# lmb-freiburg/demon

Hardware: NVIDIA H100
Metric: image_pairs_per_sec_256x192 (higher is better)
Workload: dtype tf32x3

## Files before the change

### demon_b200/csrc/conv_tc_halo.cu

```cuda
#include <cuda.h>

#include <algorithm>
#include <cstring>
#include <memory>
#include <mutex>
#include <vector>

#include "conv_tc.cuh"
#include "conv_tc_ptx.cuh"
#include "wgmma_tf32.cuh"

namespace demon {

namespace {

constexpr int kRing = 4;
constexpr int kThreads = 384;
constexpr int kConsumerWarps = 8;
constexpr int kMaxAStages = 4;
constexpr int kTileH = 16, kTileW = 8;
constexpr int kMaxPlanes = 4;
constexpr int kPlanSms = 132;
constexpr int kSmemBudget = 224 * 1024;
constexpr int kMaxDynSmem = 226 * 1024;
// ... 30 lines not shown
  int w_resident;
  int cls_bytes;
  int n_tile, nsplit;
  int mode;
  const unsigned char* w;
  float* out;
  int out_pitch, Ho, Wo, Hfull, Wfull, osy, osx, Cout;
  int cls_ooy[4], cls_oox[4];
  const float* bias;
  int leaky;
  int* err;
  long long* timing;
};

struct HaloMaps {
  CUtensorMap m[kMaxPlanes];
};

__device__ __forceinline__ void wait_t(uint32_t bar, uint32_t parity, int* err, long long& acc) {
  if (mbar_try(bar, parity)) return;
  const long long t0 = clock64();
  for (;;) {
    if (mbar_try(bar, parity)) break;
    if (clock64() - t0 > kTimeoutCycles || *reinterpret_cast<volatile int*>(err) != 0) {
      atomicExch(err, 1);
      break;
    }
  }
  acc += clock64() - t0;
}

__device__ __forceinline__ int fast_div(int x, int d, uint32_t mul) { return mul ? (int)__umulhi((uint32_t)x, mul) : x; }

template <bool PER_TAP>
__device__ __forceinline__ void halo_decode_tile(const HaloParams& p, int tile, int& nt, int& n, int& y0, int& x0) {
  int m = fast_div(tile, p.n_tiles, p.mul_n_tiles);
  nt = tile - m * p.n_tiles;
  const int m1 = fast_div(m, p.tiles_x, p.mul_tiles_x);
  const int xb = m - m1 * p.tiles_x;
  n = fast_div(m1, p.tiles_y, p.mul_tiles_y);
  const int yb = m1 - n * p.tiles_y;
  if (PER_TAP) { n *= p.tb; y0 = yb * p.th; x0 = xb * p.tw; }
  else { y0 = yb * kTileH; x0 = xb * kTileW; }
}

template <int N, int MODE>
__device__ __forceinline__ void issue_block(float* acc, const uint32_t* hi, const uint32_t* lo, uint32_t wb) {
  const uint64_t w_hi = wgmma_desc_sw128(wb);
  const uint64_t w_lo = wgmma_desc_sw128(wb + N * 128u);
#pragma unroll
  for (int j = 0; j < 4; ++j) {
    if (MODE == 2) {
      Wgmma<N>::mma(acc, hi[4 * j], hi[4 * j + 1], hi[4 * j + 2], hi[4 * j + 3], w_lo + (uint64_t)(2 * j));
      Wgmma<N>::mma(acc, lo[4 * j], lo[4 * j + 1], lo[4 * j + 2], lo[4 * j + 3], w_hi + (uint64_t)(2 * j));
    }
    Wgmma<N>::mma(acc, hi[4 * j], hi[4 * j + 1], hi[4 * j + 2], hi[4 * j + 3], w_hi + (uint64_t)(2 * j));
  }
}

template <bool PER_TAP, bool CIN8, int MODE, int N, int NCLS>
__global__ void __launch_bounds__(kThreads, 1) conv_tc_halo_kernel(const __grid_constant__ HaloMaps maps, const HaloParams p) {
  extern __shared__ __align__(1024) unsigned char smem_raw[];
  unsigned char* smem = reinterpret_cast<unsigned char*>((reinterpret_cast<uintptr_t>(smem_raw) + 1023) & ~(uintptr_t)1023);
  __shared__ __align__(8) uint64_t bars[2 * kMaxAStages + 2 * kRing + 1];

  const int warp = threadIdx.x >> 5;
  const int lane = threadIdx.x & 31;
  const uint32_t afull0 = smem_u32(&bars[0]), aempty0 = smem_u32(&bars[kMaxAStages]);
  const uint32_t wfull0 = smem_u32(&bars[2 * kMaxAStages]), wempty0 = smem_u32(&bars[2 * kMaxAStages + kRing]);
  const uint32_t wres_bar = smem_u32(&bars[2 * kMaxAStages + 2 * kRing]);
  const int a_stage_bytes = p.a_region_bytes;
  unsigned char* w_ring = smem + (size_t)p.sa * a_stage_bytes;

  if (warp == 0 && lane == 0) {
    for (int i = 0; i < p.nplanes; ++i) asm volatile("prefetch.tensormap [%0];" ::"l"(&maps.m[i]) : "memory");
    for (int s = 0; s < kMaxAStages; ++s) {
      mbar_init(afull0 + 8 * s, 1);
      mbar_init(aempty0 + 8 * s, kConsumerWarps);
    }
    for (int s = 0; s < kRing; ++s) {
      mbar_init(wfull0 + 8 * s, 1);
      mbar_init(wempty0 + 8 * s, kConsumerWarps);
    }
    mbar_init(wres_bar, 1);
    fence_barrier_init();
  }
  __syncthreads();
  const bool timed = p.timing != nullptr;
  pdl_launch_dependents();

  if (warp < 4) {
    asm volatile("setmaxnreg.dec.sync.aligned.u32 40;");
    if (warp != 0 || !elect_one_sync()) return;
    long long w_aempty = 0, w_wempty = 0;
    const long long t_begin = clock64();
    if (p.w_resident) {
      const uint32_t total = (uint32_t)(p.k_chunks * p.w_chunk_bytes);
      mbar_expect_tx(wres_bar, total);
      for (int kc = 0; kc < p.k_chunks; ++kc)
        bulk_load(smem_u32(w_ring + (size_t)kc * p.w_chunk_bytes), p.w + (size_t)kc * p.w_chunk_bytes, (uint32_t)p.w_chunk_bytes, wres_bar);
    }
    uint32_t a_bytes = 0;
    for (int i = 0; i < p.nplanes; ++i) a_bytes += (uint32_t)p.planes[i].bytes;
    int sa = 0, slot = 0;
    uint32_t pa = 0, use = 0;
    pdl_wait();
    for (int item = blockIdx.x; item < p.total_items; item += gridDim.x) {
      const int tile = fast_div(item, p.ksplit, p.mul_ksplit);
      const int kc0 = (item - tile * p.ksplit) * p.kc_split;
      int nt, n, y0, x0;
      halo_decode_tile<PER_TAP>(p, tile, nt, n, y0, x0);
      const unsigned char* wsrc = p.w + ((size_t)nt * p.k_chunks + kc0) * p.w_chunk_bytes;
      for (int kc = kc0; kc < kc0 + p.kc_split; ++kc, wsrc += p.w_chunk_bytes) {
        if (!PER_TAP) {
          wait_t(aempty0 + 8 * sa, pa ^ 1, p.err, w_aempty);
          const uint32_t abase = smem_u32(smem + (size_t)sa * a_stage_bytes);
          mbar_expect_tx(afull0 + 8 * sa, a_bytes);
          for (int i = 0; i < p.nplanes; ++i) {
            const HaloPlane& pl = p.planes[i];
            tma_load_5d(abase + pl.smem_off, &maps.m[i], afull0 + 8 * sa, pl.c_off + kc * 32, x0 + pl.qx_min, pl.ry, y0 + pl.qy_min, n);
          }
          if (++sa == p.sa) { sa = 0; pa ^= 1; }
        }
        for (int t = 0; t < p.nsteps; ++t) {
          if (PER_TAP) {
            wait_t(aempty0 + 8 * sa, pa ^ 1, p.err, w_aempty);
            mbar_expect_tx(afull0 + 8 * sa, 128u * 128u);
            tma_load_5d(smem_u32(smem + (size_t)sa * a_stage_bytes), &maps.m[0], afull0 + 8 * sa, p.tap_c[t] + kc * 32, x0 + p.tap_qx[t],
                        p.tap_ry[t], y0 + p.tap_qy[t], n);
            if (++sa == p.sa) { sa = 0; pa ^= 1; }
          }
          if (!p.w_resident) {
            wait_t(wempty0 + 8 * slot, use ^ 1, p.err, w_wempty);
            const uint32_t bytes = (uint32_t)p.st_wbytes[t];
            mbar_expect_tx(wfull0 + 8 * slot, bytes);
            bulk_load(smem_u32(w_ring + (size_t)slot * p.w_stage_bytes), wsrc + p.st_woff[t], bytes, wfull0 + 8 * slot);
            if (++slot == kRing) { slot = 0; use ^= 1; }
          }
        }
      }
    }
    if (timed) { p.timing[blockIdx.x * 16 + 0] = w_aempty; p.timing[blockIdx.x * 16 + 1] = w_wempty; p.timing[blockIdx.x * 16 + 8] = clock64() - t_begin; }
    return;
  }

  asm volatile("setmaxnreg.inc.sync.aligned.u32 232;");
  const int wg = (warp >> 2) - 1;
  const int wq = warp & 3;
  const int g = lane >> 2, tq = lane & 3;
  const int m0 = 64 * wg + 16 * wq + g;
  int pos_y[2], pos_x[2], pos_n[2];
#pragma unroll
  for (int h = 0; h < 2; ++h) {
    const int m = m0 + 8 * h;
    pos_x[h] = PER_TAP ? (m % p.tw) : (m & 7);
    pos_y[h] = PER_TAP ? ((m / p.tw) % p.th) : (m >> 3);
    pos_n[h] = PER_TAP ? (m / (p.tw * p.th)) : 0;
  }
  const float slope = p.leaky ? 0.1f : 1.0f;
  const uint32_t w_ring_u = smem_u32(w_ring);
  long long w_afull = 0, w_wfull = 0;
  const long long t_begin = clock64();
  int sa = 0, slot = 0, l_res = 0;
  uint32_t pa = 0, use = 0;
  if (p.w_resident) wait_t(wres_bar, 0u, p.err, w_wfull);
  pdl_wait();
  float acc[NCLS][N / 2];
  for (int item = blockIdx.x; item < p.total_items; item += gridDim.x) {
    const int tile = fast_div(item, p.ksplit, p.mul_ksplit);
    const int z = item - tile * p.ksplit;
    int nt, n, y0, x0;
    halo_decode_tile<PER_TAP>(p, tile, nt, n, y0, x0);
#pragma unroll
    for (int k = 0; k < NCLS; ++k)
#pragma unroll
      for (int i = 0; i < N / 2; ++i) acc[k][i] = 0.f;
    l_res = 0;
    for (int kc = 0; kc < p.kc_split; ++kc) {
      uint32_t abase = 0;
      if (!PER_TAP) {
        wait_t(afull0 + 8 * sa, pa, p.err, w_afull);
        abase = smem_u32(smem + (size_t)sa * a_stage_bytes);
      }
      for (int t = 0; t < p.nsteps; ++t) {
        if (PER_TAP) {
          wait_t(afull0 + 8 * sa, pa, p.err, w_afull);
          abase = smem_u32(smem + (size_t)sa * a_stage_bytes);
        }
        float v[2][8];
#pragma unroll
        for (int h = 0; h < 2; ++h) {
          if (CIN8) {
            const int rt = 4 * t + tq;
            const int pi = (rt < p.ntaps_real) ? p.g_plane[rt] : -1;
            float4 a = make_float4(0.f, 0.f, 0.f, 0.f), b = a;
            if (pi >= 0) {
              const HaloPlane& pl = p.planes[pi];
              const uint32_t px = abase + (uint32_t)(pl.smem_off + p.g_aoff[rt] + (pos_y[h] * pl.cols + pos_x[h]) * 32);
              a = lds128(px); b = lds128(px + 16);
            }
            v[h][0] = a.x; v[h][1] = a.y; v[h][2] = a.z; v[h][3] = a.w; v[h][4] = b.x; v[h][5] = b.y; v[h][6] = b.z; v[h][7] = b.w;
          } else {
            uint32_t row;
            if (PER_TAP) {
              row = abase + (uint32_t)((m0 + 8 * h) * 128);
            } else {
              const HaloPlane& pl = p.planes[p.st_plane[t]];
              row = abase + (uint32_t)(pl.smem_off + p.st_aoff[t] + (pos_y[h] * pl.cols + pos_x[h]) * 128);
            }
            const uint32_t phase = (row >> 7) & 7u;
            const float4 a = lds128(row + (((uint32_t)(2 * tq) ^ phase) << 4));
            const float4 b = lds128(row + (((uint32_t)(2 * tq + 1) ^ phase) << 4));
            v[h][0] = a.x; v[h][1] = a.y; v[h][2] = a.z; v[h][3] = a.w; v[h][4] = b.x; v[h][5] = b.y; v[h][6] = b.z; v[h][7] = b.w;
          }
        }
        uint32_t hi[16], lo[16];
#pragma unroll
        for (int j = 0; j < 4; ++j) {
          const float f[4] = {v[0][2 * j], v[1][2 * j], v[0][2 * j + 1], v[1][2 * j + 1]};
#pragma unroll
          for (int e = 0; e < 4; ++e) {
            const uint32_t u = __float_as_uint(f[e]);
            hi[4 * j + e] = (MODE == 2) ? (u & 0xFFFFE000u) : u;
            lo[4 * j + e] = __float_as_uint(f[e] - __uint_as_float(u & 0xFFFFE000u));
          }
        }
        uint32_t wb;
        if (p.w_resident) {
          wb = w_ring_u + (uint32_t)(l_res++) * (uint32_t)p.w_stage_bytes;
        } else {
          wait_t(wfull0 + 8 * slot, use, p.err, w_wfull);
          wb = w_ring_u + (uint32_t)slot * (uint32_t)p.w_stage_bytes;
        }
#pragma unroll
        for (int k = 0; k < NCLS; ++k)
#pragma unroll
          for (int i = 0; i < N / 2; ++i) reg_fence(acc[k][i]);
        wgmma_fence();
        if (NCLS == 1) {
          issue_block<N, MODE>(acc[0], hi, lo, wb);
        } else {
          const uint32_t cm = (uint32_t)p.st_cmask[t];
#pragma unroll
          for (int k = 0; k < NCLS; ++k)
            if (cm & (1u << k)) {
              issue_block<N, MODE>(acc[k], hi, lo, wb);
              wb += (uint32_t)p.cls_bytes;
            }
        }
        wgmma_commit();
        wgmma_wait0();
#pragma unroll
        for (int k = 0; k < NCLS; ++k)
#pragma unroll
          for (int i = 0; i < N / 2; ++i) reg_fence(acc[k][i]);
        __syncwarp();
        if (lane == 0) {
          if (!p.w_resident) mbar_arrive(wempty0 + 8 * slot);
          if (PER_TAP) mbar_arrive(aempty0 + 8 * sa);
        }
        if (!p.w_resident && ++slot == kRing) { slot = 0; use ^= 1; }
        if (PER_TAP && ++sa == p.sa) { sa = 0; pa ^= 1; }
      }
      if (!PER_TAP) {
        __syncwarp();
        if (lane == 0) mbar_arrive(aempty0 + 8 * sa);
        if (++sa == p.sa) { sa = 0; pa ^= 1; }
      }
    }
    float* tile_out = p.out + (size_t)z * p.part_stride + ((size_t)(n * p.Hfull + y0 * p.osy) * p.Wfull + x0 * p.osx) * p.out_pitch;
    const int cbase = nt * N;
#pragma unroll
    for (int k = 0; k < NCLS; ++k) {
      if (k >= p.nclass) break;
      float* cls_out = tile_out + (size_t)(p.cls_ooy[k] * p.Wfull + p.cls_oox[k]) * p.out_pitch;
#pragma unroll
      for (int h = 0; h < 2; ++h) {
        if (y0 + pos_y[h] >= p.Ho || x0 + pos_x[h] >= p.Wo || n + pos_n[h] >= p.B) continue;
        float* orow = cls_out + ((size_t)(pos_n[h] * p.Hfull + pos_y[h] * p.osy) * p.Wfull + pos_x[h] * p.osx) * p.out_pitch;
#pragma unroll
        for (int i = 0; i < N / 8; ++i) {
          const int col = cbase + 8 * i + 2 * tq;
          if (col >= p.Cout) continue;
          const float2 b = p.bias ? __ldg(reinterpret_cast<const float2*>(p.bias + col)) : make_float2(0.f, 0.f);
          float2 o;
          o.x = acc[k][4 * i + 2 * h] + b.x;
          o.y = acc[k][4 * i + 2 * h + 1] + b.y;
          o.x = fmaxf(slope * o.x, o.x); o.y = fmaxf(slope * o.y, o.y);
          *reinterpret_cast<float2*>(orow + col) = o;
        }
      }
    }
  }
  if (timed && threadIdx.x == 128) { p.timing[blockIdx.x * 16 + 6] = w_afull; p.timing[blockIdx.x * 16 + 3] = w_wfull; p.timing[blockIdx.x * 16 + 9] = clock64() - t_begin; }
}

__global__ void __launch_bounds__(256) halo_splitk_reduce_kernel(const float* __restrict__ part, long long part_stride, int ksplit,
                                                                 float* __restrict__ out, int out_pitch, int cpitch, int Cout, long long npix,
                                                                 const float* __restrict__ bias, int leaky) {
  pdl_launch_dependents();
  pdl_wait();
  const int c4n = cpitch >> 2;
  const long long total = npix * c4n;
  const float slope = leaky ? 0.1f : 1.0f;
  for (long long i = (long long)blockIdx.x * 256 + threadIdx.x; i < total; i += (long long)gridDim.x * 256) {
    const long long pix = i / c4n;
    const int c = (int)(i - pix * c4n) * 4;
    if (c >= Cout) continue;
    float4 acc = __ldg(reinterpret_cast<const float4*>(bias + c));
    for (int z = 0; z < ksplit; ++z) {
      const float4 v = *reinterpret_cast<const float4*>(part + (size_t)z * part_stride + (size_t)pix * cpitch + c);
      acc.x += v.x; acc.y += v.y; acc.z += v.z; acc.w += v.w;
    }
    acc.x = fmaxf(slope * acc.x, acc.x); acc.y = fmaxf(slope * acc.y, acc.y);
    acc.z = fmaxf(slope * acc.z, acc.z); acc.w = fmaxf(slope * acc.w, acc.w);
    *reinterpret_cast<float4*>(out + (size_t)pix * out_pitch + c) = acc;
  }
}

int floor_div_h(int a, int b) { return (a >= 0) ? a / b : -((-a + b - 1) / b); }

}

struct HaloPlan {
  HaloParams prm;
  HaloMaps maps;
  int smem_bytes;
  int st_tap[kMaxTaps][4];
};

static int pow2_ceil_h(int v) { int r = 1; while (r < v) r <<= 1; return r; }
static int popcount4(int m) { return (m & 1) + ((m >> 1) & 1) + ((m >> 2) & 1) + ((m >> 3) & 1); }

struct ShiftStep { int ry, rx, qy, qx, cmask, tap[4]; };

static bool halo_build(const ConvProblem* probs, int nclass, int nsplit, HaloPlan& plan, bool force_per_tap) {
  const ConvProblem& p = probs[0];
  HaloParams& prm = plan.prm;
  const int budget = kSmemBudget;
  struct Cand { int max_cls, n_cap; };
  std::vector<Cand> cands;
  for (int mc = nclass; mc >= 1; mc = (mc > 2 ? 2 : mc - 1)) cands.push_back({mc, 256});
  cands.push_back({1, 64});
  cands.push_back({1, 32});
  bool found = false;
  for (const Cand& cand : cands) {
    const int max_cls = cand.max_cls;
    memset(&prm, 0, sizeof(prm));
    memset(plan.st_tap, -1, sizeof(plan.st_tap));
    prm.nclass = nclass;
    prm.nsplit = nsplit;
    prm.cin8 = (p.Cin == 8) ? 1 : 0;
    const int px_bytes = prm.cin8 ? 32 : 128;
    prm.per_tap = (force_per_tap || (p.Ho % kTileH) != 0 || (p.Wo % kTileW) != 0) ? 1 : 0;
    if (prm.cin8 && (prm.per_tap || nclass != 1)) return false;
    std::vector<ShiftStep> steps;
    for (int c = 0; c < nclass; ++c)
      for (int i = 0; i < probs[c].ntaps; ++i) {
        const int qy = floor_div_h(probs[c].dy[i], p.sy), ry = probs[c].dy[i] - qy * p.sy;
        const int qx = floor_div_h(probs[c].dx[i], p.sx), rx = probs[c].dx[i] - qx * p.sx;
        int si = -1;
        for (size_t k = 0; k < steps.size(); ++k)
          if (steps[k].ry == ry && steps[k].rx == rx && steps[k].qy == qy && steps[k].qx == qx && !((steps[k].cmask >> c) & 1) &&
              popcount4(steps[k].cmask) < max_cls) { si = (int)k; break; }
        if (si < 0) { steps.push_back({ry, rx, qy, qx, 0, {-1, -1, -1, -1}}); si = (int)steps.size() - 1; }
        steps[si].cmask |= 1 << c;
        steps[si].tap[c] = i;
      }
    const int nreal = (int)steps.size();
    if (nreal > kMaxTaps) return false;
    int m_tiles = 0;
    if (prm.per_tap) {
      for (int t = 0; t < nreal; ++t) {
        prm.tap_qy[t] = steps[t].qy; prm.tap_ry[t] = steps[t].ry;
        prm.tap_qx[t] = steps[t].qx; prm.tap_c[t] = steps[t].rx * p.in_pitch;
      }
      prm.nplanes = 1;
      long best_tiles = -1;
      const int tw = std::min(128, pow2_ceil_h(p.Wo));
      for (int th = 1; th * tw <= 128; th <<= 1) {
        const int tb = 128 / (tw * th);
        const long tiles = (long)ceil_div(p.Wo, tw) * ceil_div(p.Ho, th) * ceil_div(p.B, tb);
        if (best_tiles < 0 || tiles <= best_tiles) {
          best_tiles = tiles;
          prm.tw = tw; prm.th = th; prm.tb = tb;
          prm.tiles_x = ceil_div(p.Wo, tw); prm.tiles_y = ceil_div(p.Ho, th); prm.tiles_b = ceil_div(p.B, tb);
        }
      }
      prm.planes[0].cols = prm.tw; prm.planes[0].rows = prm.th; prm.planes[0].bytes = 128 * 128;
      prm.a_region_bytes = 128 * 128;
      m_tiles = prm.tiles_x * prm.tiles_y * prm.tiles_b;
    } else {
      struct PInfo { int ry, rx, qy_min, qy_max, qx_min, qx_max; };
      std::vector<PInfo> pinfo;
      std::vector<int> step_plane(nreal);
      for (int t = 0; t < nreal; ++t) {
        int pi = -1;
        for (size_t k = 0; k < pinfo.size(); ++k)
          if (pinfo[k].ry == steps[t].ry && pinfo[k].rx == steps[t].rx) pi = (int)k;
        if (pi < 0) { pinfo.push_back({steps[t].ry, steps[t].rx, steps[t].qy, steps[t].qy, steps[t].qx, steps[t].qx}); pi = (int)pinfo.size() - 1; }
        PInfo& pl = pinfo[pi];
        pl.qy_min = std::min(pl.qy_min, steps[t].qy); pl.qy_max = std::max(pl.qy_max, steps[t].qy);
        pl.qx_min = std::min(pl.qx_min, steps[t].qx); pl.qx_max = std::max(pl.qx_max, steps[t].qx);
        step_plane[t] = pi;
      }
      if ((int)pinfo.size() > kMaxPlanes) return false;
      prm.nplanes = (int)pinfo.size();
      int off = 0;
      for (int i = 0; i < prm.nplanes; ++i) {
        HaloPlane& pl = prm.planes[i];
        pl.c_off = pinfo[i].rx * p.in_pitch; pl.ry = pinfo[i].ry;
        pl.qx_min = pinfo[i].qx_min; pl.qy_min = pinfo[i].qy_min;
        pl.cols = kTileW + pinfo[i].qx_max - pinfo[i].qx_min;
        pl.rows = kTileH + pinfo[i].qy_max - pinfo[i].qy_min;
        if (pl.cols > 256 || pl.rows > 256) return false;
        pl.bytes = pl.rows * pl.cols * px_bytes;
        pl.smem_off = off;
        off += (pl.bytes + 1023) / 1024 * 1024;
      }
      prm.a_region_bytes = off;
      for (int t = 0; t < nreal; ++t) {
        const HaloPlane& pl = prm.planes[step_plane[t]];
        prm.st_plane[t] = step_plane[t];
        prm.st_aoff[t] = ((steps[t].qy - pl.qy_min) * pl.cols + (steps[t].qx - pl.qx_min)) * px_bytes;
      }
      prm.tiles_x = ceil_div(p.Wo, kTileW); prm.tiles_y = ceil_div(p.Ho, kTileH); prm.tiles_b = p.B;
      m_tiles = prm.tiles_x * prm.tiles_y * p.B;
    }
    for (int t = 0; t < nreal; ++t) {
      prm.st_cmask[t] = steps[t].cmask;
      for (int c = 0; c < 4; ++c) plan.st_tap[t][c] = steps[t].tap[c];
    }
    prm.nsteps = nreal;
    if (prm.cin8) {
      prm.ntaps_real = nreal;
      for (int t = 0; t < nreal; ++t) { prm.g_plane[t] = prm.st_plane[t]; prm.g_aoff[t] = prm.st_aoff[t]; }
      prm.nsteps = (nreal + 3) / 4;
      for (int t = 0; t < prm.nsteps; ++t) { prm.st_plane[t] = 0; prm.st_aoff[t] = 0; prm.st_cmask[t] = 1; }
    }
    const int cout16 = (p.Cout + 15) / 16 * 16;
    int n_tile = std::min(pow2_ceil_h(std::max(cout16, 16)), std::min(nclass > 1 ? 64 : 128, cand.n_cap));
    while (n_tile >= 128 && (long)m_tiles * ceil_div(p.Cout, n_tile) < kPlanSms) n_tile /= 2;
    prm.mode = (nsplit == 1) ? 0 : 2;
    prm.n_tile = n_tile;
    prm.n_tiles = ceil_div(p.Cout, n_tile);
    prm.k_chunks = prm.cin8 ? 1 : p.Cin / 32;
    prm.cls_bytes = (nsplit == 3) ? n_tile * 256 : (n_tile * 128 + 1023) / 1024 * 1024;
    int woff = 0, wmax = 0;
    for (int t = 0; t < prm.nsteps; ++t) {
      prm.st_woff[t] = woff;
      prm.st_wbytes[t] = popcount4(prm.st_cmask[t]) * prm.cls_bytes;
      woff += prm.st_wbytes[t];
      wmax = std::max(wmax, prm.st_wbytes[t]);
    }
    prm.w_chunk_bytes = woff;
    prm.w_stage_bytes = wmax;
    const int w_total = prm.k_chunks * prm.w_chunk_bytes;
    prm.w_resident = 0;
    prm.w_region_bytes = kRing * wmax;
// ... 24 lines not shown
    for (int ks = 2; ks <= 8; ++ks) {
      if (prm.k_chunks % ks != 0 || prm.k_chunks / ks < 2) continue;
      const long c = cost(ks);
      if (c * 10 < best * 9 && c < cost(prm.ksplit)) prm.ksplit = ks;
    }
  }
  prm.kc_split = prm.k_chunks / prm.ksplit;
  prm.total_items = prm.total_tiles * prm.ksplit;
  prm.part_stride = 0;
  auto fd = [](int d) { return d <= 1 ? 0u : (uint32_t)((1ull << 32) / (uint64_t)d + 1ull); };
  prm.mul_n_tiles = fd(prm.n_tiles); prm.mul_tiles_x = fd(prm.tiles_x); prm.mul_tiles_y = fd(prm.tiles_y);
  prm.mul_ksplit = fd(prm.ksplit);
  if ((uint64_t)prm.total_items * (uint64_t)prm.ksplit >= (1ull << 32)) return false;
  if ((uint64_t)prm.total_tiles * (uint64_t)std::max(prm.n_tiles, std::max(prm.tiles_x, prm.tiles_y)) >= (1ull << 32)) return false;
  prm.out = p.out; prm.out_pitch = p.out_pitch; prm.Ho = p.Ho; prm.Wo = p.Wo; prm.Hfull = p.Hfull; prm.Wfull = p.Wfull;
  prm.osy = p.osy; prm.osx = p.osx; prm.Cout = p.Cout; prm.bias = p.bias; prm.leaky = p.leaky;
  for (int c = 0; c < nclass; ++c) { prm.cls_ooy[c] = probs[c].ooy; prm.cls_oox[c] = probs[c].oox; }
  return true;
}

static bool tc_shape_supported(const ConvProblem& p) {
  const bool cin8 = p.Cin == 8 && p.in_pitch == 8;
  if (!cin8 && (p.Cin < 32 || (p.Cin % 32) != 0)) return false;
  if (p.Cout < 16 || (p.Cout % 4) != 0) return false;
  if ((p.in_pitch % 4) != 0 || (p.out_pitch % 4) != 0) return false;
  if ((reinterpret_cast<uintptr_t>(p.in) & 15) != 0 || (reinterpret_cast<uintptr_t>(p.out) & 15) != 0) return false;
  if (p.sy < 1 || p.sx < 1 || (p.Hi % p.sy) != 0 || (p.Wi % p.sx) != 0) return false;
  if (p.ntaps < 1 || p.ntaps > kMaxTaps) return false;
  if (p.scale != nullptr) return false;
  if (p.Ho != p.Hi / p.sy || p.Wo != p.Wi / p.sx) return false;
  return true;
}

static bool tc_plan(const ConvProblem* probs, int nclass, int nsplit, HaloPlan& plan) {
  if (nclass < 1 || nclass > 4) return false;
  for (int c = 0; c < nclass; ++c) {
    if (!tc_shape_supported(probs[c])) return false;
    if (probs[c].in != probs[0].in || probs[c].Cout != probs[0].Cout || probs[c].sy != probs[0].sy || probs[c].sx != probs[0].sx) return false;
  }
  return halo_build(probs, nclass, nsplit, plan, false) || halo_build(probs, nclass, nsplit, plan, true);
}

static int nsplit_of(int precision) { return (precision == DEMON_PREC_TF32) ? 1 : 3; }

static bool encode_maps(const ConvProblem& p, HaloPlan& plan) {
  const HaloParams& prm = plan.prm;
  typedef CUresult (*EncodeTiledFn)(CUtensorMap*, CUtensorMapDataType, cuuint32_t, void*, const cuuint64_t*, const cuuint64_t*,
                                    const cuuint32_t*, const cuuint32_t*, CUtensorMapInterleave, CUtensorMapSwizzle,
                                    CUtensorMapL2promotion, CUtensorMapFloatOOBfill);
  void* fp = nullptr;
  cudaDriverEntryPointQueryResult qres;
  if (cudaGetDriverEntryPoint("cuTensorMapEncodeTiled", &fp, cudaEnableDefault, &qres) != cudaSuccess || qres != cudaDriverEntryPointSuccess)
    return false;
  EncodeTiledFn enc = reinterpret_cast<EncodeTiledFn>(fp);
  const cuuint64_t cp = (cuuint64_t)p.in_pitch;
  cuuint64_t gdim[5] = {(cuuint64_t)(p.sx - 1) * cp + (cuuint64_t)p.Cin, (cuuint64_t)(p.Wi / p.sx), (cuuint64_t)p.sy,
                        (cuuint64_t)(p.Hi / p.sy), (cuuint64_t)p.B};
  cuuint64_t gstr[4] = {(cuuint64_t)p.sx * cp * 4, (cuuint64_t)p.Wi * cp * 4, (cuuint64_t)p.sy * p.Wi * cp * 4,
                        (cuuint64_t)p.Hi * p.Wi * cp * 4};
  cuuint32_t estr[5] = {1, 1, 1, 1, 1};
  for (int i = 0; i < prm.nplanes; ++i) {
    cuuint32_t box[5] = {(cuuint32_t)(prm.cin8 ? 8 : 32), (cuuint32_t)prm.planes[i].cols, 1, (cuuint32_t)prm.planes[i].rows,
                         (cuuint32_t)(prm.per_tap ? prm.tb : 1)};
    CUresult r = enc(&plan.maps.m[i], CU_TENSOR_MAP_DATA_TYPE_FLOAT32, 5, const_cast<float*>(p.in), gdim, gstr, box, estr,
                     CU_TENSOR_MAP_INTERLEAVE_NONE, prm.cin8 ? CU_TENSOR_MAP_SWIZZLE_NONE : CU_TENSOR_MAP_SWIZZLE_128B,
                     CU_TENSOR_MAP_L2_PROMOTION_L2_256B, CU_TENSOR_MAP_FLOAT_OOB_FILL_NONE);
    if (r != CUDA_SUCCESS) return false;
  }
  for (int i = prm.nplanes; i < kMaxPlanes; ++i) plan.maps.m[i] = plan.maps.m[0];
  return true;
}

int tc_describe(const ConvProblem* probs, int nclass, int precision, char* buf, int buflen) {
  HaloPlan plan;
  if (!tc_plan(probs, nclass, nsplit_of(precision), plan)) return 0;
  const HaloParams& q = plan.prm;
  int n = snprintf(buf, buflen, "halo %s mode %d n_tile %d x%d steps %d x %d chunks sa %d a_stage %d w_slot %d smem %d tiles %d ksplit %d wres %d |",
                   q.per_tap ? "per-tap" : (q.cin8 ? "cin8" : "halo"), q.mode, q.n_tile, q.n_tiles, q.nsteps, q.k_chunks, q.sa,
                   q.a_region_bytes, q.w_stage_bytes, plan.smem_bytes, q.total_tiles, q.ksplit, q.w_resident);
  for (int t = 0; t < q.nsteps && n < buflen - 32; ++t)
    n += snprintf(buf + n, buflen - n, " [c%x w%d+%d]", q.st_cmask[t], q.st_woff[t], q.st_wbytes[t]);
  return n;
}

static float tf32_round_h(float x) {
  uint32_t u;
  memcpy(&u, &x, 4);
  if ((u & 0x7F800000u) == 0x7F800000u) return x;
  u += 0x00000FFFu + ((u >> 13) & 1u);
  u &= 0xFFFFE000u;
  float r;
  memcpy(&r, &u, 4);
  return r;
}

int tc_prepare(TcLayer& t, const ConvProblem* probs, const float* const* w_hosts, int nclass, int precision) {
  const ConvProblem& p = probs[0];
  const int nsplit = nsplit_of(precision);
  std::unique_ptr<HaloPlan> plan(new HaloPlan());
  if (!tc_plan(probs, nclass, nsplit, *plan)) return kTcNoPlan;
  if (!encode_maps(p, *plan)) return fail(DEMON_E_CUDA, "tc_prepare: tensor map encode failed");
  const HaloParams& prm = plan->prm;
  const size_t total = (size_t)prm.n_tiles * prm.k_chunks * prm.w_chunk_bytes;
  std::vector<unsigned char> packed(total, 0);
  for (int nt = 0; nt < prm.n_tiles; ++nt)
    for (int kc = 0; kc < prm.k_chunks; ++kc)
      for (int tt = 0; tt < prm.nsteps; ++tt) {
        int idx = 0;
        for (int cls = 0; cls < 4; ++cls) {
          if (!((prm.st_cmask[tt] >> cls) & 1)) continue;
          unsigned char* blk = packed.data() + ((size_t)nt * prm.k_chunks + kc) * prm.w_chunk_bytes + prm.st_woff[tt] + (size_t)idx * prm.cls_bytes;
          ++idx;
// ... 58 lines not shown
  if (s.device != dev) {
    s = TcDeviceState();
    s.device = dev;
    int sms = 0;
    cudaDeviceGetAttribute(&sms, cudaDevAttrMultiProcessorCount, dev);
    s.sms = sms > 0 ? sms : 132;
    if (cudaMalloc(&s.err_dev, sizeof(int)) == cudaSuccess) cudaMemset(s.err_dev, 0, sizeof(int));
    else s.err_dev = nullptr;
  }
  return s;
}

int tc_read_error_flag(bool clear) {
  TcDeviceState& ds = tc_device_state();
  if (!ds.err_dev) return 0;
  int v = 0;
  cudaMemcpy(&v, ds.err_dev, sizeof(int), cudaMemcpyDeviceToHost);
  if (v && clear) cudaMemset(ds.err_dev, 0, sizeof(int));
  return v;
}

static long long* g_timing_dev = nullptr;
void tc_halo_enable_timing(bool on) {
  if (on && !g_timing_dev) { cudaMalloc(&g_timing_dev, 256 * 16 * sizeof(long long)); }
  if (g_timing_dev) cudaMemset(g_timing_dev, 0, 256 * 16 * sizeof(long long));
  if (!on && g_timing_dev) { cudaFree(g_timing_dev); g_timing_dev = nullptr; }
}
int tc_halo_read_timing(long long* host, int nblocks) {
  if (!g_timing_dev) return -1;
  cudaMemcpy(host, g_timing_dev, (size_t)nblocks * 16 * sizeof(long long), cudaMemcpyDeviceToHost);
  return 0;
}

template <bool PER_TAP, bool CIN8, int MODE, int N, int NCLS>
static int launch_variant(const HaloPlan* plan, const HaloParams& prm, int grid, cudaStream_t stream) {
  TcDeviceState& ds = tc_device_state();
  static int attr_device = -1;
  if (attr_device != ds.device) {
    DEMON_CHECK_CUDA(cudaFuncSetAttribute(conv_tc_halo_kernel<PER_TAP, CIN8, MODE, N, NCLS>, cudaFuncAttributeMaxDynamicSharedMemorySize, kMaxDynSmem));
    attr_device = ds.device;
  }
  cudaError_t le = launch_pdl(conv_tc_halo_kernel<PER_TAP, CIN8, MODE, N, NCLS>, dim3(grid), dim3(kThreads), (size_t)plan->smem_bytes, stream, plan->maps, prm);
  if (le != cudaSuccess) return fail(DEMON_E_CUDA, "conv_tc_halo launch: %s", cudaGetErrorString(le));
  DEMON_LAUNCH_CHECK();
  return DEMON_OK;
}

template <bool PER_TAP, bool CIN8, int MODE, int NCLS>
static int launch_n(const HaloPlan* plan, const HaloParams& prm, int grid, cudaStream_t stream) {
  switch (prm.n_tile) {
    case 16: return launch_variant<PER_TAP, CIN8, MODE, 16, NCLS>(plan, prm, grid, stream);
    case 32: return launch_variant<PER_TAP, CIN8, MODE, 32, NCLS>(plan, prm, grid, stream);
    case 64: return launch_variant<PER_TAP, CIN8, MODE, 64, NCLS>(plan, prm, grid, stream);
    default: break;
  }
  if (NCLS == 1 && prm.n_tile == 128) return launch_variant<PER_TAP, CIN8, MODE, (NCLS == 1 ? 128 : 64), NCLS>(plan, prm, grid, stream);
  return fail(DEMON_E_STATE, "conv_tc_halo: no kernel for N tile %d with %d classes", prm.n_tile, prm.nclass);
}

template <bool PER_TAP, bool CIN8, int NCLS>
static int launch_mode(const HaloPlan* plan, const HaloParams& prm, int grid, cudaStream_t stream) {
  return prm.mode == 0 ? launch_n<PER_TAP, CIN8, 0, NCLS>(plan, prm, grid, stream) : launch_n<PER_TAP, CIN8, 2, NCLS>(plan, prm, grid, stream);
}

int conv_tc_launch(const TcLayer& t, const ConvProblem* probs, cudaStream_t stream) {
  const HaloPlan* plan = t.plan;
  HaloParams prm = plan->prm;
  prm.out = probs[0].out;
  prm.out_pitch = probs[0].out_pitch;
  TcDeviceState& ds = tc_device_state();
  if (!ds.err_dev) return fail(DEMON_E_CUDA, "tensor-core path: no error flag on device %d", ds.device);
  prm.err = ds.err_dev;
  prm.timing = g_timing_dev;
  const int cpitch = (prm.Cout + 3) / 4 * 4;
  const long long npix = (long long)prm.B * prm.Hfull * prm.Wfull;
  float* const final_out = prm.out;
  const int final_pitch = prm.out_pitch;
  if (prm.ksplit > 1) {
    if (!probs[0].partial) return fail(DEMON_E_STATE, "conv_tc_halo: split-K layer launched without a scratch buffer");
    prm.out = probs[0].partial;
    prm.out_pitch = cpitch;
    prm.part_stride = npix * cpitch;
    prm.bias = nullptr;
    prm.leaky = 0;
  }
  const int grid = std::min(prm.total_items, ds.sms);
  int rc;
  if (prm.cin8) rc = launch_mode<false, true, 1>(plan, prm, grid, stream);
  else if (prm.per_tap) rc = prm.nclass == 1 ? launch_mode<true, false, 1>(plan, prm, grid, stream) : launch_mode<true, false, 4>(plan, prm, grid, stream);
  else rc = prm.nclass == 1 ? launch_mode<false, false, 1>(plan, prm, grid, stream) : launch_mode<false, false, 4>(plan, prm, grid, stream);
  if (rc != DEMON_OK || prm.ksplit == 1) return rc;
  const long long total = npix * (cpitch / 4);
  const int blocks = (int)std::min<long long>((total + 255) / 256, (long long)ds.sms * 8);
  cudaError_t le = launch_pdl(halo_splitk_reduce_kernel, dim3(blocks), dim3(256), 0, stream, (const float*)probs[0].partial, prm.part_stride,
                              prm.ksplit, final_out, final_pitch, cpitch, prm.Cout, npix, plan->prm.bias, plan->prm.leaky);
  if (le != cudaSuccess) return fail(DEMON_E_CUDA, "halo_splitk_reduce launch: %s", cudaGetErrorString(le));
  DEMON_LAUNCH_CHECK();
  return DEMON_OK;
}

}
```

### demon_b200/csrc/conv_tc_ptx.cuh

```cuda
#pragma once
#include <cuda.h>
#include <cstdint>

namespace demon {
namespace {

constexpr long long kTimeoutCycles = 4000000000ll;

__device__ __forceinline__ uint32_t smem_u32(const void* p) { return (uint32_t)__cvta_generic_to_shared(p); }

__device__ __forceinline__ void mbar_init(uint32_t bar, uint32_t count) {
  asm volatile("mbarrier.init.shared::cta.b64 [%0], %1;" ::"r"(bar), "r"(count));
}
__device__ __forceinline__ void mbar_arrive(uint32_t bar) {
  asm volatile("{\n.reg .b64 st;\nmbarrier.arrive.shared::cta.b64 st, [%0];\n}" ::"r"(bar) : "memory");
}
__device__ __forceinline__ void mbar_expect_tx(uint32_t bar, uint32_t bytes) {
  asm volatile("{\n.reg .b64 st;\nmbarrier.arrive.expect_tx.shared::cta.b64 st, [%0], %1;\n}" ::"r"(bar), "r"(bytes) : "memory");
}
__device__ __forceinline__ bool mbar_try(uint32_t bar, uint32_t parity) {
  uint32_t done;
  asm volatile(
      "{\n.reg .pred p;\n"
      "mbarrier.try_wait.parity.shared::cta.b64 p, [%1], %2;\n"
      "selp.u32 %0, 1, 0, p;\n}"
      : "=r"(done)
      : "r"(bar), "r"(parity)
      : "memory");
  return done != 0;
}
__device__ __forceinline__ void fence_barrier_init() { asm volatile("fence.mbarrier_init.release.cluster;" ::: "memory"); }
__device__ __forceinline__ void tma_load_5d(uint32_t dst, const CUtensorMap* map, uint32_t bar, int c0, int c1, int c2, int c3, int c4) {
  asm volatile(
      "cp.async.bulk.tensor.5d.shared::cluster.global.mbarrier::complete_tx::bytes [%0], [%1, {%3, %4, %5, %6, %7}], [%2];"
      ::"r"(dst), "l"(map), "r"(bar), "r"(c0), "r"(c1), "r"(c2), "r"(c3), "r"(c4)
      : "memory");
}
__device__ __forceinline__ void bulk_load(uint32_t dst, const void* src, uint32_t bytes, uint32_t bar) {
  asm volatile("cp.async.bulk.shared::cluster.global.mbarrier::complete_tx::bytes [%0], [%1], %2, [%3];" ::"r"(dst), "l"(src),
               "r"(bytes), "r"(bar)
               : "memory");
}
__device__ __forceinline__ void wgmma_fence() { asm volatile("wgmma.fence.sync.aligned;" ::: "memory"); }
__device__ __forceinline__ void wgmma_commit() { asm volatile("wgmma.commit_group.sync.aligned;" ::: "memory"); }
__device__ __forceinline__ void wgmma_wait0() { asm volatile("wgmma.wait_group.sync.aligned 0;" ::: "memory"); }
__device__ __forceinline__ void reg_fence(float& x) { asm volatile("" : "+f"(x)::"memory"); }

__device__ __forceinline__ uint64_t wgmma_desc_sw128(uint32_t smem_addr) {
  uint64_t d = 0;
  d |= (uint64_t)((smem_addr & 0x3FFFF) >> 4);
  d |= (uint64_t)1 << 16;
  d |= (uint64_t)(1024 >> 4) << 32;
  d |= (uint64_t)1 << 62;
  return d;
}

__device__ __forceinline__ bool elect_one_sync() {
  uint32_t pred;
  asm volatile("{\n.reg .b32 rx;\n.reg .pred px;\nelect.sync rx|px, 0xffffffff;\nselp.b32 %0, 1, 0, px;\n}" : "=r"(pred));
  return pred != 0;
}

__device__ __forceinline__ float4 lds128(uint32_t addr) {
  float4 v;
  asm volatile("ld.shared.v4.f32 {%0, %1, %2, %3}, [%4];" : "=f"(v.x), "=f"(v.y), "=f"(v.z), "=f"(v.w) : "r"(addr));
  return v;
}
}
}
```

Before: 2050.

## Add two-block-wide halo tiles so each consumer reuses weights across two M blocks

Adds an MB=2 variant of the halo conv kernel in which each tile is twice as wide (16 columns). Each consumer warpgroup then keeps two 64-row accumulator sets and issues wgmma for both against the same weight descriptor, so every staged weight slice is reused across twice as many pixels. The planner picks this variant only for single-class, non-per-tap layers with N≤64 and enough tiles and pipeline stages. The cost is doubled accumulator and fragment registers, larger A stages that may reduce the stage count, and fewer tiles for load balancing.

New measurement: 2106, median of 6. 2.8% higher.

```diff
diff --git a/demon_b200/csrc/conv_tc_halo.cu b/demon_b200/csrc/conv_tc_halo.cu
--- a/demon_b200/csrc/conv_tc_halo.cu
+++ b/demon_b200/csrc/conv_tc_halo.cu
@@ -86,7 +86,7 @@
 
 __device__ __forceinline__ int fast_div(int x, int d, uint32_t mul) { return mul ? (int)__umulhi((uint32_t)x, mul) : x; }
 
-template <bool PER_TAP>
+template <bool PER_TAP, int TW>
 __device__ __forceinline__ void halo_decode_tile(const HaloParams& p, int tile, int& nt, int& n, int& y0, int& x0) {
   int m = fast_div(tile, p.n_tiles, p.mul_n_tiles);
   nt = tile - m * p.n_tiles;
@@ -95,7 +95,16 @@
   n = fast_div(m1, p.tiles_y, p.mul_tiles_y);
   const int yb = m1 - n * p.tiles_y;
   if (PER_TAP) { n *= p.tb; y0 = yb * p.th; x0 = xb * p.tw; }
-  else { y0 = yb * kTileH; x0 = xb * kTileW; }
+  else { y0 = yb * kTileH; x0 = xb * TW; }
+}
+
+template <int N, int MODE>
+__device__ __forceinline__ void issue_slice(float* acc, const uint32_t* hi, const uint32_t* lo, uint64_t w_hi, uint64_t w_lo, int j) {
+  if (MODE == 2) {
+    Wgmma<N>::mma(acc, hi[4 * j], hi[4 * j + 1], hi[4 * j + 2], hi[4 * j + 3], w_lo + (uint64_t)(2 * j));
+    Wgmma<N>::mma(acc, lo[4 * j], lo[4 * j + 1], lo[4 * j + 2], lo[4 * j + 3], w_hi + (uint64_t)(2 * j));
+  }
+  Wgmma<N>::mma(acc, hi[4 * j], hi[4 * j + 1], hi[4 * j + 2], hi[4 * j + 3], w_hi + (uint64_t)(2 * j));
 }
 
 template <int N, int MODE>
@@ -103,17 +112,13 @@
   const uint64_t w_hi = wgmma_desc_sw128(wb);
   const uint64_t w_lo = wgmma_desc_sw128(wb + N * 128u);
 #pragma unroll
-  for (int j = 0; j < 4; ++j) {
-    if (MODE == 2) {
-      Wgmma<N>::mma(acc, hi[4 * j], hi[4 * j + 1], hi[4 * j + 2], hi[4 * j + 3], w_lo + (uint64_t)(2 * j));
-      Wgmma<N>::mma(acc, lo[4 * j], lo[4 * j + 1], lo[4 * j + 2], lo[4 * j + 3], w_hi + (uint64_t)(2 * j));
-    }
-    Wgmma<N>::mma(acc, hi[4 * j], hi[4 * j + 1], hi[4 * j + 2], hi[4 * j + 3], w_hi + (uint64_t)(2 * j));
-  }
-}
-
-template <bool PER_TAP, bool CIN8, int MODE, int N, int NCLS>
+  for (int j = 0; j < 4; ++j) issue_slice<N, MODE>(acc, hi, lo, w_hi, w_lo, j);
+}
+
+template <bool PER_TAP, bool CIN8, int MODE, int N, int NCLS, int MB>
 __global__ void __launch_bounds__(kThreads, 1) conv_tc_halo_kernel(const __grid_constant__ HaloMaps maps, const HaloParams p) {
+  static_assert(MB == 1 || (MB == 2 && !PER_TAP && !CIN8 && NCLS == 1 && N <= 64), "MB = 2: one-class halo mode, N <= 64");
+  constexpr int TW = kTileW * MB;
   extern __shared__ __align__(1024) unsigned char smem_raw[];
   unsigned char* smem = reinterpret_cast<unsigned char*>((reinterpret_cast<uintptr_t>(smem_raw) + 1023) & ~(uintptr_t)1023);
   __shared__ __align__(8) uint64_t bars[2 * kMaxAStages + 2 * kRing + 1];
@@ -163,7 +168,7 @@
       const int tile = fast_div(item, p.ksplit, p.mul_ksplit);
       const int kc0 = (item - tile * p.ksplit) * p.kc_split;
       int nt, n, y0, x0;
-      halo_decode_tile<PER_TAP>(p, tile, nt, n, y0, x0);
+      halo_decode_tile<PER_TAP, TW>(p, tile, nt, n, y0, x0);
       const unsigned char* wsrc = p.w + ((size_t)nt * p.k_chunks + kc0) * p.w_chunk_bytes;
       for (int kc = kc0; kc < kc0 + p.kc_split; ++kc, wsrc += p.w_chunk_bytes) {
         if (!PER_TAP) {
@@ -203,14 +208,22 @@
   const int wq = warp & 3;
   const int g = lane >> 2, tq = lane & 3;
   const int m0 = 64 * wg + 16 * wq + g;
-  int pos_y[2], pos_x[2], pos_n[2];
-#pragma unroll
-  for (int h = 0; h < 2; ++h) {
-    const int m = m0 + 8 * h;
-    pos_x[h] = PER_TAP ? (m % p.tw) : (m & 7);
-    pos_y[h] = PER_TAP ? ((m / p.tw) % p.th) : (m >> 3);
-    pos_n[h] = PER_TAP ? (m / (p.tw * p.th)) : 0;
-  }
+  int pos_y[MB][2], pos_x[MB][2], pos_n[MB][2];
+#pragma unroll
+  for (int bk = 0; bk < MB; ++bk)
+#pragma unroll
+    for (int h = 0; h < 2; ++h) {
+      if (MB == 1) {
+        const int m = m0 + 8 * h;
+        pos_x[bk][h] = PER_TAP ? (m % p.tw) : (m & 7);
+        pos_y[bk][h] = PER_TAP ? ((m / p.tw) % p.th) : (m >> 3);
+        pos_n[bk][h] = PER_TAP ? (m / (p.tw * p.th)) : 0;
+      } else {
+        pos_x[bk][h] = g + 8 * h;
+        pos_y[bk][h] = 8 * wg + 4 * bk + wq;
+        pos_n[bk][h] = 0;
+      }
+    }
   const float slope = p.leaky ? 0.1f : 1.0f;
   const uint32_t w_ring_u = smem_u32(w_ring);
   long long w_afull = 0, w_wfull = 0;
@@ -219,14 +232,14 @@
   uint32_t pa = 0, use = 0;
   if (p.w_resident) wait_t(wres_bar, 0u, p.err, w_wfull);
   pdl_wait();
-  float acc[NCLS][N / 2];
+  float acc[NCLS * MB][N / 2];
   for (int item = blockIdx.x; item < p.total_items; item += gridDim.x) {
     const int tile = fast_div(item, p.ksplit, p.mul_ksplit);
     const int z = item - tile * p.ksplit;
     int nt, n, y0, x0;
-    halo_decode_tile<PER_TAP>(p, tile, nt, n, y0, x0);
-#pragma unroll
-    for (int k = 0; k < NCLS; ++k)
+    halo_decode_tile<PER_TAP, TW>(p, tile, nt, n, y0, x0);
+#pragma unroll
+    for (int k = 0; k < NCLS * MB; ++k)
 #pragma unroll
       for (int i = 0; i < N / 2; ++i) acc[k][i] = 0.f;
     l_res = 0;
@@ -241,44 +254,50 @@
           wait_t(afull0 + 8 * sa, pa, p.err, w_afull);
           abase = smem_u32(smem + (size_t)sa * a_stage_bytes);
         }
-        float v[2][8];
-#pragma unroll
-        for (int h = 0; h < 2; ++h) {
-          if (CIN8) {
-            const int rt = 4 * t + tq;
-            const int pi = (rt < p.ntaps_real) ? p.g_plane[rt] : -1;
-            float4 a = make_float4(0.f, 0.f, 0.f, 0.f), b = a;
-            if (pi >= 0) {
-              const HaloPlane& pl = p.planes[pi];
-              const uint32_t px = abase + (uint32_t)(pl.smem_off + p.g_aoff[rt] + (pos_y[h] * pl.cols + pos_x[h]) * 32);
-              a = lds128(px); b = lds128(px + 16);
+        float v[MB][2][8];
+#pragma unroll
+        for (int bk = 0; bk < MB; ++bk)
+#pragma unroll
+          for (int h = 0; h < 2; ++h) {
+            if (CIN8) {
+              const int rt = 4 * t + tq;
+              const int pi = (rt < p.ntaps_real) ? p.g_plane[rt] : -1;
+              float4 a = make_float4(0.f, 0.f, 0.f, 0.f), b = a;
+              if (pi >= 0) {
+                const HaloPlane& pl = p.planes[pi];
+                const uint32_t px = abase + (uint32_t)(pl.smem_off + p.g_aoff[rt] + (pos_y[bk][h] * pl.cols + pos_x[bk][h]) * 32);
+                a = lds128(px); b = lds128(px + 16);
+              }
+              v[bk][h][0] = a.x; v[bk][h][1] = a.y; v[bk][h][2] = a.z; v[bk][h][3] = a.w;
+              v[bk][h][4] = b.x; v[bk][h][5] = b.y; v[bk][h][6] = b.z; v[bk][h][7] = b.w;
+            } else {
+              uint32_t row;
+              if (PER_TAP) {
+                row = abase + (uint32_t)((m0 + 8 * h) * 128);
+              } else {
+                const HaloPlane& pl = p.planes[p.st_plane[t]];
+                row = abase + (uint32_t)(pl.smem_off + p.st_aoff[t] + (pos_y[bk][h] * pl.cols + pos_x[bk][h]) * 128);
+              }
+              const uint32_t phase = (row >> 7) & 7u;
+              const float4 a = lds128(row + (((uint32_t)(2 * tq) ^ phase) << 4));
+              const float4 b = lds128(row + (((uint32_t)(2 * tq + 1) ^ phase) << 4));
+              v[bk][h][0] = a.x; v[bk][h][1] = a.y; v[bk][h][2] = a.z; v[bk][h][3] = a.w;
+              v[bk][h][4] = b.x; v[bk][h][5] = b.y; v[bk][h][6] = b.z; v[bk][h][7] = b.w;
             }
-            v[h][0] = a.x; v[h][1] = a.y; v[h][2] = a.z; v[h][3] = a.w; v[h][4] = b.x; v[h][5] = b.y; v[h][6] = b.z; v[h][7] = b.w;
-          } else {
-            uint32_t row;
-            if (PER_TAP) {
-              row = abase + (uint32_t)((m0 + 8 * h) * 128);
-            } else {
-              const HaloPlane& pl = p.planes[p.st_plane[t]];
-              row = abase + (uint32_t)(pl.smem_off + p.st_aoff[t] + (pos_y[h] * pl.cols + pos_x[h]) * 128);
+          }
+        uint32_t hi[MB][16], lo[MB][16];
+#pragma unroll
+        for (int bk = 0; bk < MB; ++bk)
+#pragma unroll
+          for (int j = 0; j < 4; ++j) {
+            const float f[4] = {v[bk][0][2 * j], v[bk][1][2 * j], v[bk][0][2 * j + 1], v[bk][1][2 * j + 1]};
+#pragma unroll
+            for (int e = 0; e < 4; ++e) {
+              const uint32_t u = __float_as_uint(f[e]);
+              hi[bk][4 * j + e] = (MODE == 2) ? (u & 0xFFFFE000u) : u;
+              lo[bk][4 * j + e] = __float_as_uint(f[e] - __uint_as_float(u & 0xFFFFE000u));
             }
-            const uint32_t phase = (row >> 7) & 7u;
-            const float4 a = lds128(row + (((uint32_t)(2 * tq) ^ phase) << 4));
-            const float4 b = lds128(row + (((uint32_t)(2 * tq + 1) ^ phase) << 4));
-            v[h][0] = a.x; v[h][1] = a.y; v[h][2] = a.z; v[h][3] = a.w; v[h][4] = b.x; v[h][5] = b.y; v[h][6] = b.z; v[h][7] = b.w;
           }
-        }
-        uint32_t hi[16], lo[16];
-#pragma unroll
-        for (int j = 0; j < 4; ++j) {
-          const float f[4] = {v[0][2 * j], v[1][2 * j], v[0][2 * j + 1], v[1][2 * j + 1]};
-#pragma unroll
-          for (int e = 0; e < 4; ++e) {
-            const uint32_t u = __float_as_uint(f[e]);
-            hi[4 * j + e] = (MODE == 2) ? (u & 0xFFFFE000u) : u;
-            lo[4 * j + e] = __float_as_uint(f[e] - __uint_as_float(u & 0xFFFFE000u));
-          }
-        }
         uint32_t wb;
         if (p.w_resident) {
           wb = w_ring_u + (uint32_t)(l_res++) * (uint32_t)p.w_stage_bytes;
@@ -287,25 +306,39 @@
           wb = w_ring_u + (uint32_t)slot * (uint32_t)p.w_stage_bytes;
         }
 #pragma unroll
-        for (int k = 0; k < NCLS; ++k)
+        for (int k = 0; k < NCLS * MB; ++k)
 #pragma unroll
           for (int i = 0; i < N / 2; ++i) reg_fence(acc[k][i]);
+#pragma unroll
+        for (int bk = 0; bk < MB; ++bk)
+#pragma unroll
+          for (int i = 0; i < 16; ++i) {
+            reg_fence_u(hi[bk][i]);
+            if (MODE == 2) reg_fence_u(lo[bk][i]);
+          }
         wgmma_fence();
-        if (NCLS == 1) {
-          issue_block<N, MODE>(acc[0], hi, lo, wb);
+        if (MB == 2) {
+          const uint64_t w_hi = wgmma_desc_sw128(wb);
+          const uint64_t w_lo = wgmma_desc_sw128(wb + N * 128u);
+#pragma unroll
+          for (int j = 0; j < 4; ++j)
+#pragma unroll
+            for (int bk = 0; bk < MB; ++bk) issue_slice<N, MODE>(acc[bk], hi[bk], lo[bk], w_hi, w_lo, j);
+        } else if (NCLS == 1) {
+          issue_block<N, MODE>(acc[0], hi[0], lo[0], wb);
         } else {
           const uint32_t cm = (uint32_t)p.st_cmask[t];
 #pragma unroll
           for (int k = 0; k < NCLS; ++k)
             if (cm & (1u << k)) {
-              issue_block<N, MODE>(acc[k], hi, lo, wb);
+              issue_block<N, MODE>(acc[k], hi[0], lo[0], wb);
               wb += (uint32_t)p.cls_bytes;
             }
         }
         wgmma_commit();
         wgmma_wait0();
 #pragma unroll
-        for (int k = 0; k < NCLS; ++k)
+        for (int k = 0; k < NCLS * MB; ++k)
 #pragma unroll
           for (int i = 0; i < N / 2; ++i) reg_fence(acc[k][i]);
         __syncwarp();
@@ -329,21 +362,23 @@
       if (k >= p.nclass) break;
       float* cls_out = tile_out + (size_t)(p.cls_ooy[k] * p.Wfull + p.cls_oox[k]) * p.out_pitch;
 #pragma unroll
-      for (int h = 0; h < 2; ++h) {
-        if (y0 + pos_y[h] >= p.Ho || x0 + pos_x[h] >= p.Wo || n + pos_n[h] >= p.B) continue;
-        float* orow = cls_out + ((size_t)(pos_n[h] * p.Hfull + pos_y[h] * p.osy) * p.Wfull + pos_x[h] * p.osx) * p.out_pitch;
-#pragma unroll
-        for (int i = 0; i < N / 8; ++i) {
-          const int col = cbase + 8 * i + 2 * tq;
-          if (col >= p.Cout) continue;
-          const float2 b = p.bias ? __ldg(reinterpret_cast<const float2*>(p.bias + col)) : make_float2(0.f, 0.f);
-          float2 o;
-          o.x = acc[k][4 * i + 2 * h] + b.x;
-          o.y = acc[k][4 * i + 2 * h + 1] + b.y;
-          o.x = fmaxf(slope * o.x, o.x); o.y = fmaxf(slope * o.y, o.y);
-          *reinterpret_cast<float2*>(orow + col) = o;
+      for (int bk = 0; bk < MB; ++bk)
+#pragma unroll
+        for (int h = 0; h < 2; ++h) {
+          if (y0 + pos_y[bk][h] >= p.Ho || x0 + pos_x[bk][h] >= p.Wo || n + pos_n[bk][h] >= p.B) continue;
+          float* orow = cls_out + ((size_t)(pos_n[bk][h] * p.Hfull + pos_y[bk][h] * p.osy) * p.Wfull + pos_x[bk][h] * p.osx) * p.out_pitch;
+#pragma unroll
+          for (int i = 0; i < N / 8; ++i) {
+            const int col = cbase + 8 * i + 2 * tq;
+            if (col >= p.Cout) continue;
+            const float2 b = p.bias ? __ldg(reinterpret_cast<const float2*>(p.bias + col)) : make_float2(0.f, 0.f);
+            float2 o;
+            o.x = acc[k * MB + bk][4 * i + 2 * h] + b.x;
+            o.y = acc[k * MB + bk][4 * i + 2 * h + 1] + b.y;
+            o.x = fmaxf(slope * o.x, o.x); o.y = fmaxf(slope * o.y, o.y);
+            *reinterpret_cast<float2*>(orow + col) = o;
+          }
         }
-      }
     }
   }
   if (timed && threadIdx.x == 128) { p.timing[blockIdx.x * 16 + 6] = w_afull; p.timing[blockIdx.x * 16 + 3] = w_wfull; p.timing[blockIdx.x * 16 + 9] = clock64() - t_begin; }
@@ -380,6 +415,7 @@
   HaloParams prm;
   HaloMaps maps;
   int smem_bytes;
+  int mb;
   int st_tap[kMaxTaps][4];
 };
 
@@ -388,10 +424,12 @@
 
 struct ShiftStep { int ry, rx, qy, qx, cmask, tap[4]; };
 
-static bool halo_build(const ConvProblem* probs, int nclass, int nsplit, HaloPlan& plan, bool force_per_tap) {
+static bool halo_build(const ConvProblem* probs, int nclass, int nsplit, HaloPlan& plan, bool force_per_tap, int mb = 1) {
   const ConvProblem& p = probs[0];
   HaloParams& prm = plan.prm;
   const int budget = kSmemBudget;
+  const int tile_w = kTileW * mb;
+  plan.mb = mb;
   struct Cand { int max_cls, n_cap; };
   std::vector<Cand> cands;
   for (int mc = nclass; mc >= 1; mc = (mc > 2 ? 2 : mc - 1)) cands.push_back({mc, 256});
@@ -406,7 +444,7 @@
     prm.nsplit = nsplit;
     prm.cin8 = (p.Cin == 8) ? 1 : 0;
     const int px_bytes = prm.cin8 ? 32 : 128;
-    prm.per_tap = (force_per_tap || (p.Ho % kTileH) != 0 || (p.Wo % kTileW) != 0) ? 1 : 0;
+    prm.per_tap = (force_per_tap || (p.Ho % kTileH) != 0 || (p.Wo % tile_w) != 0) ? 1 : 0;
     if (prm.cin8 && (prm.per_tap || nclass != 1)) return false;
     std::vector<ShiftStep> steps;
     for (int c = 0; c < nclass; ++c)
@@ -465,7 +503,7 @@
         HaloPlane& pl = prm.planes[i];
         pl.c_off = pinfo[i].rx * p.in_pitch; pl.ry = pinfo[i].ry;
         pl.qx_min = pinfo[i].qx_min; pl.qy_min = pinfo[i].qy_min;
-        pl.cols = kTileW + pinfo[i].qx_max - pinfo[i].qx_min;
+        pl.cols = tile_w + pinfo[i].qx_max - pinfo[i].qx_min;
         pl.rows = kTileH + pinfo[i].qy_max - pinfo[i].qy_min;
         if (pl.cols > 256 || pl.rows > 256) return false;
         pl.bytes = pl.rows * pl.cols * px_bytes;
@@ -478,7 +516,7 @@
         prm.st_plane[t] = step_plane[t];
         prm.st_aoff[t] = ((steps[t].qy - pl.qy_min) * pl.cols + (steps[t].qx - pl.qx_min)) * px_bytes;
       }
-      prm.tiles_x = ceil_div(p.Wo, kTileW); prm.tiles_y = ceil_div(p.Ho, kTileH); prm.tiles_b = p.B;
+      prm.tiles_x = ceil_div(p.Wo, tile_w); prm.tiles_y = ceil_div(p.Ho, kTileH); prm.tiles_b = p.B;
       m_tiles = prm.tiles_x * prm.tiles_y * p.B;
     }
     for (int t = 0; t < nreal; ++t) {
@@ -569,13 +607,30 @@
   return true;
 }
 
+constexpr int kMb2MinWaves = 4;
+constexpr int kMb2MinStepsN64 = 16;
 static bool tc_plan(const ConvProblem* probs, int nclass, int nsplit, HaloPlan& plan) {
   if (nclass < 1 || nclass > 4) return false;
   for (int c = 0; c < nclass; ++c) {
     if (!tc_shape_supported(probs[c])) return false;
     if (probs[c].in != probs[0].in || probs[c].Cout != probs[0].Cout || probs[c].sy != probs[0].sy || probs[c].sx != probs[0].sx) return false;
   }
-  return halo_build(probs, nclass, nsplit, plan, false) || halo_build(probs, nclass, nsplit, plan, true);
+  if (halo_build(probs, nclass, nsplit, plan, false)) {
+    const HaloParams& q = plan.prm;
+    if (nclass == 1 && !q.per_tap && !q.cin8 && (q.n_tile <= 32 || (q.n_tile == 64 && q.nsteps * q.k_chunks >= kMb2MinStepsN64)) &&
+        q.ksplit == 1 && (probs[0].Ho % kTileH) == 0 &&
+        (probs[0].Wo % (2 * kTileW)) == 0) {
+      std::unique_ptr<HaloPlan> wide(new HaloPlan());
+      if (halo_build(probs, nclass, nsplit, *wide, false, 2)) {
+        const HaloParams& w = wide->prm;
+        if (!w.per_tap && w.n_tile == q.n_tile && w.w_resident == q.w_resident && w.sa >= 2 && w.ksplit == 1 &&
+            w.total_tiles >= kMb2MinWaves * kPlanSms)
+          plan = *wide;
+      }
+    }
+    return true;
+  }
+  return halo_build(probs, nclass, nsplit, plan, true);
 }
 
 static int nsplit_of(int precision) { return (precision == DEMON_PREC_TF32) ? 1 : 3; }
@@ -612,9 +667,9 @@
   HaloPlan plan;
   if (!tc_plan(probs, nclass, nsplit_of(precision), plan)) return 0;
   const HaloParams& q = plan.prm;
-  int n = snprintf(buf, buflen, "halo %s mode %d n_tile %d x%d steps %d x %d chunks sa %d a_stage %d w_slot %d smem %d tiles %d ksplit %d wres %d |",
+  int n = snprintf(buf, buflen, "halo %s mode %d n_tile %d x%d steps %d x %d chunks sa %d a_stage %d w_slot %d smem %d tiles %d ksplit %d wres %d mb %d |",
                    q.per_tap ? "per-tap" : (q.cin8 ? "cin8" : "halo"), q.mode, q.n_tile, q.n_tiles, q.nsteps, q.k_chunks, q.sa,
-                   q.a_region_bytes, q.w_stage_bytes, plan.smem_bytes, q.total_tiles, q.ksplit, q.w_resident);
+                   q.a_region_bytes, q.w_stage_bytes, plan.smem_bytes, q.total_tiles, q.ksplit, q.w_resident, plan.mb);
   for (int t = 0; t < q.nsteps && n < buflen - 32; ++t)
     n += snprintf(buf + n, buflen - n, " [c%x w%d+%d]", q.st_cmask[t], q.st_woff[t], q.st_wbytes[t]);
   return n;
@@ -739,35 +794,36 @@
   return 0;
 }
 
-template <bool PER_TAP, bool CIN8, int MODE, int N, int NCLS>
+template <bool PER_TAP, bool CIN8, int MODE, int N, int NCLS, int MB>
 static int launch_variant(const HaloPlan* plan, const HaloParams& prm, int grid, cudaStream_t stream) {
   TcDeviceState& ds = tc_device_state();
   static int attr_device = -1;
   if (attr_device != ds.device) {
-    DEMON_CHECK_CUDA(cudaFuncSetAttribute(conv_tc_halo_kernel<PER_TAP, CIN8, MODE, N, NCLS>, cudaFuncAttributeMaxDynamicSharedMemorySize, kMaxDynSmem));
+    DEMON_CHECK_CUDA(cudaFuncSetAttribute(conv_tc_halo_kernel<PER_TAP, CIN8, MODE, N, NCLS, MB>, cudaFuncAttributeMaxDynamicSharedMemorySize, kMaxDynSmem));
     attr_device = ds.device;
   }
-  cudaError_t le = launch_pdl(conv_tc_halo_kernel<PER_TAP, CIN8, MODE, N, NCLS>, dim3(grid), dim3(kThreads), (size_t)plan->smem_bytes, stream, plan->maps, prm);
+  cudaError_t le = launch_pdl(conv_tc_halo_kernel<PER_TAP, CIN8, MODE, N, NCLS, MB>, dim3(grid), dim3(kThreads), (size_t)plan->smem_bytes, stream, plan->maps, prm);
   if (le != cudaSuccess) return fail(DEMON_E_CUDA, "conv_tc_halo launch: %s", cudaGetErrorString(le));
   DEMON_LAUNCH_CHECK();
   return DEMON_OK;
 }
 
-template <bool PER_TAP, bool CIN8, int MODE, int NCLS>
+template <bool PER_TAP, bool CIN8, int MODE, int NCLS, int MB>
 static int launch_n(const HaloPlan* plan, const HaloParams& prm, int grid, cudaStream_t stream) {
   switch (prm.n_tile) {
-    case 16: return launch_variant<PER_TAP, CIN8, MODE, 16, NCLS>(plan, prm, grid, stream);
-    case 32: return launch_variant<PER_TAP, CIN8, MODE, 32, NCLS>(plan, prm, grid, stream);
-    case 64: return launch_variant<PER_TAP, CIN8, MODE, 64, NCLS>(plan, prm, grid, stream);
+    case 16: return launch_variant<PER_TAP, CIN8, MODE, 16, NCLS, MB>(plan, prm, grid, stream);
+    case 32: return launch_variant<PER_TAP, CIN8, MODE, 32, NCLS, MB>(plan, prm, grid, stream);
+    case 64: return launch_variant<PER_TAP, CIN8, MODE, 64, NCLS, MB>(plan, prm, grid, stream);
     default: break;
   }
-  if (NCLS == 1 && prm.n_tile == 128) return launch_variant<PER_TAP, CIN8, MODE, (NCLS == 1 ? 128 : 64), NCLS>(plan, prm, grid, stream);
-  return fail(DEMON_E_STATE, "conv_tc_halo: no kernel for N tile %d with %d classes", prm.n_tile, prm.nclass);
-}
-
-template <bool PER_TAP, bool CIN8, int NCLS>
+  if (NCLS == 1 && MB == 1 && prm.n_tile == 128)
+    return launch_variant<PER_TAP, CIN8, MODE, (NCLS == 1 && MB == 1 ? 128 : 64), NCLS, MB>(plan, prm, grid, stream);
+  return fail(DEMON_E_STATE, "conv_tc_halo: no kernel for N tile %d with %d classes and %d blocks", prm.n_tile, prm.nclass, MB);
+}
+
+template <bool PER_TAP, bool CIN8, int NCLS, int MB = 1>
 static int launch_mode(const HaloPlan* plan, const HaloParams& prm, int grid, cudaStream_t stream) {
-  return prm.mode == 0 ? launch_n<PER_TAP, CIN8, 0, NCLS>(plan, prm, grid, stream) : launch_n<PER_TAP, CIN8, 2, NCLS>(plan, prm, grid, stream);
+  return prm.mode == 0 ? launch_n<PER_TAP, CIN8, 0, NCLS, MB>(plan, prm, grid, stream) : launch_n<PER_TAP, CIN8, 2, NCLS, MB>(plan, prm, grid, stream);
 }
 
 int conv_tc_launch(const TcLayer& t, const ConvProblem* probs, cudaStream_t stream) {
@@ -793,7 +849,8 @@
   }
   const int grid = std::min(prm.total_items, ds.sms);
   int rc;
-  if (prm.cin8) rc = launch_mode<false, true, 1>(plan, prm, grid, stream);
+  if (plan->mb == 2) rc = launch_mode<false, false, 1, 2>(plan, prm, grid, stream);
+  else if (prm.cin8) rc = launch_mode<false, true, 1>(plan, prm, grid, stream);
   else if (prm.per_tap) rc = prm.nclass == 1 ? launch_mode<true, false, 1>(plan, prm, grid, stream) : launch_mode<true, false, 4>(plan, prm, grid, stream);
   else rc = prm.nclass == 1 ? launch_mode<false, false, 1>(plan, prm, grid, stream) : launch_mode<false, false, 4>(plan, prm, grid, stream);
   if (rc != DEMON_OK || prm.ksplit == 1) return rc;
diff --git a/demon_b200/csrc/conv_tc_ptx.cuh b/demon_b200/csrc/conv_tc_ptx.cuh
--- a/demon_b200/csrc/conv_tc_ptx.cuh
+++ b/demon_b200/csrc/conv_tc_ptx.cuh
@@ -45,6 +45,7 @@
 __device__ __forceinline__ void wgmma_commit() { asm volatile("wgmma.commit_group.sync.aligned;" ::: "memory"); }
 __device__ __forceinline__ void wgmma_wait0() { asm volatile("wgmma.wait_group.sync.aligned 0;" ::: "memory"); }
 __device__ __forceinline__ void reg_fence(float& x) { asm volatile("" : "+f"(x)::"memory"); }
+__device__ __forceinline__ void reg_fence_u(uint32_t& x) { asm volatile("" : "+r"(x)::"memory"); }
 
 __device__ __forceinline__ uint64_t wgmma_desc_sw128(uint32_t smem_addr) {
   uint64_t d = 0;
```
